# frobelbest/BANet

Measured on AMD Instinct MI355X. Metric: LM iterations/sec (2-frame 640x480 5-level dense BA, 128-coeff depth basis, batch 32), higher is better.
Workload: dtype f32 (SYRK: fp32 operands as bf16x3 / scaled fp16x2 pieces, fp32 accumulate, <= 2e-7 per entry; roofline.syrk_form)

## Files before the change

banet_amd/csrc/api.hip:

```cpp
#include "kernels.hpp"

namespace banet {

static bool aligned256(const void* p) { return (reinterpret_cast<uintptr_t>(p) & 255u) == 0; }

static int check_level(const banet_level_t* lv) {
  if (!lv || !lv->src || !lv->tgt || !lv->depth) return BANET_ERR_INVALID_ARG;
  if (lv->variant < BANET_LEGACY_LM || lv->variant > BANET_BUNDLE) return BANET_ERR_INVALID_ARG;
  if (lv->K > 0 && !lv->basis) return BANET_ERR_INVALID_ARG;
  if ((lv->variant == BANET_BUNDLE) != (lv->K > 0)) return BANET_ERR_INVALID_ARG;
  if (lv->pairs < 0 || (lv->policy != BANET_POLICY_THROUGHPUT && lv->policy != BANET_POLICY_BATCH_INVARIANT)) return BANET_ERR_INVALID_ARG;
  if (lv->pairs > 1 && lv->variant != BANET_BUNDLE && lv->variant != BANET_BUNDLE_CAMERA) return BANET_ERR_INVALID_ARG;
  if (lv->dense) {
    if (!lv->intr || !(lv->scale > 0.f)) return BANET_ERR_INVALID_ARG;
  } else {
    if (!lv->rays || !lv->fx || !lv->fy || !lv->ox || !lv->oy) return BANET_ERR_INVALID_ARG;
  }
  return BANET_OK;
}

static LevelWs carve_level(const banet_level_t* lv, const AsmPlan& pl, void* ws) {
  LevelWs w;
  char* p = static_cast<char*>(ws);
  Arena ar;
// ... 58 lines not shown


constexpr int kRoleSmallLevel = 19200;

int lm_level_plan(const banet_level_t* lv, const banet_mlp_t* mlp, float l2_base, int max_iters, int early_termination,
                  const banet_lm_params_t* params, const banet_state_t* st, void* ws, size_t ws_bytes, LevelRun* run) {
  int rc = check_level(lv);
  if (rc != BANET_OK) return rc;
  rc = check_state(lv, mlp, st);
  if (rc != BANET_OK) return rc;
  if (max_iters < 0) return BANET_ERR_INVALID_ARG;
  AsmPlan& pl = run->pl;
  rc = plan_assemble(lv, num_cus(), &pl);
  if (rc != BANET_OK) return rc;
  if (!ws || !aligned256(ws)) return BANET_ERR_WORKSPACE;
  LevelWs& w = run->w;
  w = carve_level(lv, pl, ws);
  if (ws_bytes < w.total) return BANET_ERR_WORKSPACE;
  SolveArgs& a = run->a;
  a = make_solve_args(lv, mlp, l2_base, w.AtA, w.Atb, w.absres, w.nvalid, st);
  a.max_iters = max_iters;
  a.bigA = w.bigA;
  if (params) {
    if (params->solver != BANET_SOLVER_QR && params->solver != BANET_SOLVER_INVERSE) return BANET_ERR_INVALID_ARG;
    if (!(params->angle_change >= 0.f) || !(params->translation_change >= 0.f) || !(params->residual_ratio > 0.f))
      return BANET_ERR_INVALID_ARG;
    a.lm = *params;
  }
  run->lv = lv;
  run->mlp = mlp;
  run->max_iters = max_iters;
  run->lm = early_termination && lv->variant == BANET_LEGACY_LM;
  run->role = false;
  if (run->lm) {
    a.ctl = w.ctl;
  } else {
    a.queue = assemble_queue(pl, w.partials);
    a.nqueue = 8 * npairs(lv);
    const int Bsel = selection_batch(lv);
    run->role = lv->variant == BANET_BUNDLE && mlp != nullptr && a.use_mlp && syrk_runs_mlp_role(pl.s) && lv->C <= 256 &&
                (lv->C & 3) == 0 && ((long long)Bsel * (pl.s.Gs + 1) <= num_cus() || (Bsel <= 8 && pl.s.Gs >= 16) ||
                 (lv->N <= kRoleSmallLevel && pl.s.Gs >= 4)) &&
                !(lv->flags & kDevMlpInSolve);
    if (run->role) {
      a.mlp_y = w.mlp_y;
      if ((long long)Bsel * (pl.s.Gs + 1) > num_cus()) pl.s.Gs -= 1;
    }
  }
  return BANET_OK;
}

int lm_level_enqueue(const LevelRun& run, hipStream_t s) {
  const banet_level_t* lv = run.lv;
  const AsmPlan& pl = run.pl;
  const LevelWs& w = run.w;
  const SolveArgs& a = run.a;
  const banet_state_t* st = &a.st;
  const int max_iters = run.max_iters;
  int rc;
  if (run.lm) {
    launch_ctl_init(w.ctl, st->iters, lv->B, s);
    const int stride = (int)(sizeof(LmCtl) / sizeof(int32_t));
    for (int it = 0; it <= max_iters; ++it) {
      rc = launch_assemble(lv, pl, st->R, st->T, st->Wc, &w.ctl->active, stride, w.partials, w.AtA, w.Atb, w.absres,
                           w.nvalid, s);
      if (rc != BANET_OK) return rc;
      {
        RangeScope r("solve", lv->N);
        rc = launch_solve(a, s);
      }
      if (rc != BANET_OK) return rc;
    }
  } else {
    launch_zero_iters(st->iters, lv->B, s);
    if (a.queue) launch_zero_iters(a.queue, lv->B * a.nqueue, s);
    const bool role = run.role;
    const banet_mlp_t* mlp = run.mlp;
    for (int it = 0; it < max_iters; ++it) {
      rc = launch_assemble(lv, pl, st->R, st->T, st->Wc, nullptr, 0, w.partials, w.AtA, w.Atb, w.absres, w.nvalid, s,
                           a.queue == nullptr, role ? mlp : nullptr, role ? w.mlp_y : nullptr, nullptr,
                           pl.s.f16 ? (it == 0 ? (max_iters > 1 ? 2 : 0) : 1) : -1);
      if (rc != BANET_OK) return rc;
      {
        RangeScope r("solve", lv->N);
        rc = launch_solve(a, s);
      }
      if (rc != BANET_OK) return rc;
    }
  }
  return BANET_OK;
}

}

using namespace banet;

extern "C" {

int banet_version(void) { return BANET_VERSION; }

const char* banet_error_string(int code) {
  switch (code) {
    case BANET_OK: return "ok";
    case BANET_ERR_INVALID_ARG: return "invalid argument";
    case BANET_ERR_WORKSPACE: return "workspace too small or misaligned";
    case BANET_ERR_UNSUPPORTED: return "shape not supported by the compiled kernel set";
    case BANET_ERR_LAUNCH: return "kernel launch failed";
    default: return "unknown error";
  }
}

size_t banet_equation_construction_workspace_bytes(int B, int N, int C, int P) {
  EqPlan pl;
  if (plan_eq(B, N, C, P, &pl) != BANET_OK) return 0;
// ... 323 lines not shown
```

banet_amd/csrc/assemble.hip:

```cpp
#include <atomic>
#include <dlfcn.h>

#include <cstdio>
#include <cstdlib>
#include <vector>

#include "kernels.hpp"

namespace banet {

namespace {
struct Profiler {
  bool on = false;
  std::vector<hipEvent_t> ev;
  std::vector<int> tag;
  int used = 0;
} g_prof;

struct Timed {
  hipStream_t s;
  int slot;
  Timed(hipStream_t st, int tag) : s(st), slot(-1) {
    if (g_prof.on && (size_t)(2 * g_prof.used + 1) < g_prof.ev.size()) {
      slot = g_prof.used++;
// ... 87 lines not shown

int num_cus() {
  constexpr int kMaxDev = 64, kDefault = 256;
  static std::atomic<int> cached[kMaxDev];
  static const int pinned = [] {
    const char* e = std::getenv("BANET_NUM_CUS");
    const int v = e ? std::atoi(e) : 0;
    return v > 0 && v <= 4096 ? v : 0;
  }();
  if (pinned) return pinned;
  int dev = 0;
  if (hipGetDevice(&dev) != hipSuccess || dev < 0 || dev >= kMaxDev) {
    (void)hipGetLastError();
    return kDefault;
  }
  int n = cached[dev].load(std::memory_order_relaxed);
  if (n == 0) {
    if (hipDeviceGetAttribute(&n, hipDeviceAttributeMultiprocessorCount, dev) != hipSuccess || n <= 0) {
      (void)hipGetLastError();
      n = kDefault;
    }
    cached[dev].store(n, std::memory_order_relaxed);
  }
  return n;
}

int* assemble_queue(const AsmPlan& pl, void* ws) {
  return pl.g.c128 ? reinterpret_cast<int*>(static_cast<char*>(ws) + pl.g.off_queue) : nullptr;
}

int launch_assemble(const banet_level_t* lv, const AsmPlan& pl, const float* R, const float* T, const float* Wc,
                    const int32_t* active, int active_stride, void* ws, float* AtA, float* Atb, float* absres,
                    float* nvalid, hipStream_t s, bool reset_queue, const banet_mlp_t* role_mlp, float* role_y,
                    unsigned char* mask_out, int f16_stats) {
  char* base = static_cast<char*>(ws);
  float* gpart = reinterpret_cast<float*>(base);
  float* rec = lv->K > 0 ? reinterpret_cast<float*>(base + pl.off_rec) : nullptr;
  float* spart = lv->K > 0 ? reinterpret_cast<float*>(base + pl.off_spart) : nullptr;
  int rc;
  if (reset_queue) prepare_gather(lv, pl.g, gpart, s);
  {
    RangeScope r("gather", lv->N);
    Timed t(s, lv->N);
    rc = launch_gather(lv, pl.g, R, T, Wc, active, active_stride, rec, gpart, s, mask_out);
  }
  if (rc != BANET_OK) return rc;
  const float* gred;
  {
    RangeScope r("fold", lv->N);
    gred = finish_gather(lv, pl.g, active, active_stride, gpart, s);
  }
  if (lv->K > 0) {
    RangeScope r("syrk", lv->N);
    Timed t(s, -lv->N);
    MlpRole mr{};
    if (role_mlp != nullptr && role_y != nullptr && syrk_runs_mlp_role(pl.s)) {
      mr.gpart = gred;
      mr.grows = pl.g.frows;
      mr.gstride = pl.g.pstride;
      mr.mlp = *role_mlp;
      mr.C = lv->C;
      mr.pairs = npairs(lv);
      mr.Nf = (float)lv->N * (float)npairs(lv);
      mr.y = role_y;
    }
    rc = launch_syrk(lv->basis, rec, lv->B, lv->N, lv->K, npairs(lv), pl.s, active, active_stride, spart, s,
                     mr.y != nullptr ? &mr : nullptr, f16_stats);
    if (rc != BANET_OK) return rc;
  }
  RangeScope r("reduce", lv->N);
  launch_reduce2(gred, pl.g.frows, pl.g.pstride, spart, pl.s.Gs, pl.s.pstride, active, active_stride, lv->B, lv->K, lv->C,
                 npairs(lv), AtA, Atb, absres, nvalid, s);
  return hipGetLastError() == hipSuccess ? BANET_OK : BANET_ERR_LAUNCH;
}

}
```

banet_amd/csrc/gather.hip:

```cpp
#include <algorithm>
#include "gather_common.hpp"

namespace banet {

template <int VEC, int CH, bool GRAD, int KVEC, int KCH>
__global__ __launch_bounds__(kBlock, BANET_GATHER_WAVES) void ba_gather_kernel(const GatherArgs a) {
  __shared__ float sH[kNumWaves][28][64];
  __shared__ float sAbs[kNumWaves][256];
  const banet_level_t& lv = a.lv;
  const int vb = blockIdx.y, g = blockIdx.x;
  const int b = vb / a.pairs;
  if (a.active != nullptr && a.active[(size_t)b * a.active_stride] == 0) return;
  const int tid = threadIdx.x, lane = tid & 63;
  const int w = wave_id();
  const int N = lv.N, C = lv.C, K = lv.K, H = lv.H, W = lv.W;
  const int Ct = GRAD ? 3 * C : C;
  const bool dense = lv.dense != 0;
  const int dbg = lv.flags;
  const float* __restrict__ tgt_b = lv.tgt + (size_t)vb * H * W * Ct;
  const float* __restrict__ src_b = lv.src + (size_t)b * N * C;
  const float* __restrict__ dep_b = lv.depth + (size_t)b * N;
  const float* __restrict__ bas_b = KCH ? lv.basis + (size_t)b * N * K : nullptr;
  float* __restrict__ rec_b = KCH ? a.rec + (size_t)vb * N * 8 : nullptr;

#pragma unroll
  for (int i = 0; i < 28; ++i) sH[w][i][lane] = 0.f;
#ifdef BANET_TIMING
  float tim0 = 0.f, tim1 = 0.f, tim2 = 0.f, tim3 = 0.f;
#endif
  float absd[CH][VEC];
#pragma unroll
  for (int i = 0; i < CH; ++i)
#pragma unroll
    for (int e = 0; e < VEC; ++e) absd[i][e] = 0.f;
// ... 323 lines not shown
  if (tid == 0) {
    float* dp = a.partials + ((size_t)vb * a.G + g) * (kGHdr + C);
    dp[28] = tim0;
    dp[29] = tim1;
    dp[30] = tim2;
    dp[31] = tim3;
  }
#endif

#pragma unroll
  for (int ch = 0; ch < CH; ++ch)
#pragma unroll
    for (int e = 0; e < VEC; ++e) {
      const int c = (ch * 64 + lane) * VEC + e;
      if (c < C) sAbs[w][c] = absd[ch][e];
    }
  __syncthreads();
  float* __restrict__ part = a.partials + ((size_t)vb * a.G + g) * (kGHdr + C);
  if (tid < 4 * 28) {
    const int ww = tid / 28, i = tid - ww * 28;
    float s = 0.f;
    for (int l = 0; l < 64; ++l) s += sH[ww][i][l];
    sH[ww][i][0] = s;
  }
  __syncthreads();
  if (tid < 28) part[tid] = (sH[0][tid][0] + sH[1][tid][0]) + (sH[2][tid][0] + sH[3][tid][0]);
  for (int c = tid; c < C; c += kBlock) part[kGHdr + c] = (sAbs[0][c] + sAbs[1][c]) + (sAbs[2][c] + sAbs[3][c]);
}


__global__ __launch_bounds__(256) void ba_fold_kernel(const float* __restrict__ in, int rows, int stride,
                                                      float* __restrict__ out, int frows, const int32_t* active,
                                                      int active_stride, int pairs) {
  const int b = blockIdx.y, c = blockIdx.x, e = threadIdx.x;
  if (active != nullptr && active[(size_t)(b / pairs) * active_stride] == 0) return;
  if (e >= stride) return;
  const int r0 = c * kFoldRows, r1 = min(rows, r0 + kFoldRows);
  const float* p = in + ((size_t)b * rows + r0) * stride + e;
  float s0 = 0.f, s1 = 0.f, s2 = 0.f, s3 = 0.f;
  int i = 0;
  const int n = r1 - r0;
  for (; i + 3 < n; i += 4) {
    s0 += p[(size_t)(i + 0) * stride];
    s1 += p[(size_t)(i + 1) * stride];
    s2 += p[(size_t)(i + 2) * stride];
    s3 += p[(size_t)(i + 3) * stride];
  }
  for (; i < n; ++i) s0 += p[(size_t)i * stride];
  out[((size_t)b * frows + c) * stride + e] = (s0 + s1) + (s2 + s3);
}

void prepare_gather(const banet_level_t* lv, const GatherPlan& pl, float* partials, hipStream_t s) {
  if (pl.c128) launch_zero_iters(reinterpret_cast<int32_t*>(reinterpret_cast<char*>(partials) + pl.off_queue), lv->B * npairs(lv) * 8, s);
}

const float* finish_gather(const banet_level_t* lv, const GatherPlan& pl, const int32_t* active, int active_stride,
                           float* partials, hipStream_t s) {
  if (pl.frows == pl.rows) return partials;
  float* out = reinterpret_cast<float*>(reinterpret_cast<char*>(partials) + pl.off_fold);
  hipLaunchKernelGGL(ba_fold_kernel, dim3(pl.frows, lv->B * npairs(lv)), dim3(256), 0, s, partials, pl.rows, pl.pstride, out,
                     pl.frows, active, active_stride, npairs(lv));
  return out;
}

template <int VEC, int CH, bool GRAD>
static int launch_k(const GatherArgs& a, int K, hipStream_t s) {
  dim3 grid(a.G, a.lv.B * a.pairs), block(kBlock);
  const bool keven = (K & 1) == 0;
  if (K == 0)
    hipLaunchKernelGGL((ba_gather_kernel<VEC, CH, GRAD, 1, 0>), grid, block, 0, s, a);
  else if (keven && K <= 128)
    hipLaunchKernelGGL((ba_gather_kernel<VEC, CH, GRAD, 2, 1>), grid, block, 0, s, a);
  else if (keven && K <= 256)
    hipLaunchKernelGGL((ba_gather_kernel<VEC, CH, GRAD, 2, 2>), grid, block, 0, s, a);
  else if (K <= 64)
    hipLaunchKernelGGL((ba_gather_kernel<VEC, CH, GRAD, 1, 1>), grid, block, 0, s, a);
  else if (K <= 128)
    hipLaunchKernelGGL((ba_gather_kernel<VEC, CH, GRAD, 1, 2>), grid, block, 0, s, a);
  else
    return BANET_ERR_UNSUPPORTED;
  return BANET_OK;
}
// ... 47 lines not shown
```

banet_amd/csrc/kernels.hpp:

```cpp
#pragma once
#include "common.hpp"
#include "grid_plan.hpp"

namespace banet {

constexpr int kUStrideS = 8;

int num_cus();

void prepare_gather(const banet_level_t* lv, const GatherPlan& pl, float* partials, hipStream_t s);
int launch_gather(const banet_level_t* lv, const GatherPlan& pl, const float* R, const float* T, const float* Wc,
                  const int32_t* active, int active_stride, float* rec, float* partials, hipStream_t s,
                  unsigned char* mask_out = nullptr);
const float* finish_gather(const banet_level_t* lv, const GatherPlan& pl, const int32_t* active, int active_stride,
                           float* partials, hipStream_t s);

struct MlpRole {
  const float* gpart;
  int grows, gstride;
  banet_mlp_t mlp;
  int C, pairs;
  float Nf;
  float* y;
};
int launch_syrk_wide(const float* basis, const float* rec, int B, int N, int K, int pairs, int Gs, int pstride,
                     const int32_t* active, int active_stride, float* partials, float* aux, hipStream_t s,
                     const float* colmax = nullptr, const float* recmax = nullptr);
int launch_syrk(const float* basis, const float* rec, int B, int N, int K, int pairs, const SyrkPlan& pl,
                const int32_t* active, int active_stride, float* partials, hipStream_t s, const MlpRole* mr = nullptr,
                int f16_stats = -1);
inline bool syrk_runs_mlp_role(const SyrkPlan& pl) { return pl.direct == 2; }
void launch_reduce2(const float* gpart, int Gg, int gstride, const float* spart, int Gs, int sstride,
                    const int32_t* active, int active_stride, int B, int K, int C, int pairs, float* AtA, float* Atb,
                    float* absres, float* nvalid, hipStream_t s);

int launch_assemble(const banet_level_t* lv, const AsmPlan& pl, const float* R, const float* T, const float* Wc,
                    const int32_t* active, int active_stride, void* ws, float* AtA, float* Atb, float* absres,
                    float* nvalid, hipStream_t s, bool reset_queue = true, const banet_mlp_t* role_mlp = nullptr,
                    float* role_y = nullptr, unsigned char* mask_out = nullptr, int f16_stats = -1);
int* assemble_queue(const AsmPlan& pl, void* ws);
int profile_ranges(int enable);
struct RangeScope {
  bool on;
  RangeScope(const char* role, int n = -1);
  ~RangeScope();
};
int profile_begin(int max_launches);
int profile_end(int max_tags, int32_t* tag_points, int32_t* tag_launches, double* tag_ms, int32_t* ntags);

int launch_resample(const float* data, const float* warp, float* out, int B, int N, int C, int H, int W, int mode,
                    hipStream_t s);
int launch_target_map(const float* img, float* out, int B, int H, int W, int C, hipStream_t s);
int launch_depth_output(const float* init, const float* basis, const float* Wc, float* out, int B, int N, int K,
                        hipStream_t s);

bool resample_grad_supported(int B, int N, int C, int H, int W);
size_t resample_grad_workspace_bytes(int B, int N, int C, int H, int W);
int launch_resample_grad(const float* data, const float* warp, const float* gout, float* ddata, float* dwarp, int B, int N, int C, int H,
                         int W, int mode, int overwrite, void* ws, hipStream_t s);
size_t depth_output_grad_workspace_bytes(int B, int N, int K);
int launch_depth_output_grad(const float* basis, const float* Wc, const float* gout, float* dinit, float* dbasis, float* dWc, int B,
                             int N, int K, int overwrite, void* ws, hipStream_t s);

int launch_grid_resample(const float* data, int B, int H, int W, int C, int mode, const banet_grid_level_t* levels, int n_levels,
                         hipStream_t s);
int launch_grid_resample_grad(float* ddata, int B, int H, int W, int C, int mode, const banet_grid_level_t* levels, int n_levels,
                              int overwrite, hipStream_t s);

void launch_reduce(const float* partials, int B, int G, int pstride, int P, float* AtA, float* Atb, hipStream_t s);
struct EqPlan {
  int Gr, tiles, pstride, nb;
  int fast;
// ... 63 lines not shown
size_t sample_stats_grad_det_workspace_bytes(int B, int N, int C, int H, int W);
int launch_sample_stats_grad_det(const float* conv1, const float* conv2, const float* px, const float* py, int B, int N, int C,
                                 int H, int W, const float* dstats, const float* dabs, float* dconv1, float* dconv2, float* dpos,
                                 void* ws, hipStream_t s);
int launch_target_map_adjoint(const float* dmap3, float* dimg, int B, int H, int W, int C, int overwrite, hipStream_t s);

bool small_step_supported(int variant, int B, int N, int C, int K, int pairs);
size_t small_step_workspace_bytes(int variant, int B, int N, int C, int K, int pairs);
int launch_small_step_adjoint(int variant, int B, int N, int C, int K, int pairs, float l2_base, const banet_mlp_t* mlp, const float* AtA,
                              const float* Atb, const float* absres, const float* delta, const float* R, const float* T, const float* gR,
                              const float* gT, const float* gW, float* gAtA, float* gAtb, float* gabs, float* dR, float* dT,
                              const banet_mlp_t* gmlp, void* ws, hipStream_t s);

struct LevelWs {
  float* partials;
  float* AtA;
  float* Atb;
  float* absres;
  float* nvalid;
  LmCtl* ctl;
  float* mlp_y;
  float* bigA;
  size_t total;
};
struct LevelRun {
  const banet_level_t* lv;
  const banet_mlp_t* mlp;
  AsmPlan pl;
  LevelWs w;
  SolveArgs a;
  int max_iters;
  bool lm;
  bool role;
};
int lm_level_plan(const banet_level_t* lv, const banet_mlp_t* mlp, float l2_base, int max_iters, int early_termination,
                  const banet_lm_params_t* params, const banet_state_t* st, void* ws, size_t ws_bytes, LevelRun* run);
int lm_level_enqueue(const LevelRun& run, hipStream_t s);

struct TraceRow {
  banet_state_t from, to;
  int nR, nT, K, P;
};
void launch_lm_trace(const TraceRow& row, int B, hipStream_t s);

}
```

banet_amd/csrc/mlp.hpp:

```cpp
#pragma once
#include "kernels.hpp"

namespace banet {

constexpr float kSeluAlpha = 1.6732632423543772848170429916717f;
constexpr float kSeluScale = 1.0507009873554804934193349852946f;

__device__ __forceinline__ float selu(float x) {
  return kSeluScale * (x > 0.f ? x : kSeluAlpha * (expf(x) - 1.f));
}

template <int NT>
__device__ float block_sum_t(float v, float* sred) {
  v = wave_sum(v);
  __syncthreads();
  if ((threadIdx.x & 63) == 0) sred[threadIdx.x >> 6] = v;
  __syncthreads();
  float r = 0.f;
#pragma unroll
  for (int i = 0; i < NT / 64; ++i) r += sred[i];
  return r;
}

template <int NT>
__device__ void mlp_layer_t(const float* in, float* out, const float* __restrict__ Wt, const float* __restrict__ bias,
                          int nin, int nout, int act, float* sPart, float* sred) {
  const int tid = threadIdx.x;
  const int groups = nout >> 2;
  if ((nout & 3) == 0 && groups <= NT && ((reinterpret_cast<uintptr_t>(Wt) & 15) == 0)) {
    int ksplit = NT / groups;
    if (ksplit > nin) ksplit = nin;
    const int q = tid % groups, sl = tid / groups;
    if (sl < ksplit) {
      const int chunk = (nin + ksplit - 1) / ksplit;
// ... 20 lines not shown
    }
    __syncthreads();
  } else if (nout >= 64) {
    for (int o = tid; o < nout; o += NT) {
      float a0 = 0.f, a1 = 0.f, a2 = 0.f, a3 = 0.f;
      int i = 0;
      for (; i + 3 < nin; i += 4) {
        a0 = fmaf(in[i], Wt[(size_t)i * nout + o], a0);
        a1 = fmaf(in[i + 1], Wt[(size_t)(i + 1) * nout + o], a1);
        a2 = fmaf(in[i + 2], Wt[(size_t)(i + 2) * nout + o], a2);
        a3 = fmaf(in[i + 3], Wt[(size_t)(i + 3) * nout + o], a3);
      }
      for (; i < nin; ++i) a0 = fmaf(in[i], Wt[(size_t)i * nout + o], a0);
      const float v = ((a0 + a1) + (a2 + a3)) + bias[o];
      out[o] = act == 0 ? selu(v) : tanhf(v);
    }
    __syncthreads();
  } else {
    for (int o = 0; o < nout; ++o) {
      float a = 0.f;
      for (int i = tid; i < nin; i += NT) a = fmaf(in[i], Wt[(size_t)i * nout + o], a);
      const float s = block_sum_t<NT>(a, sred);
      if (tid == 0) {
        const float v = s + bias[o];
        out[o] = act == 0 ? selu(v) : tanhf(v);
      }
    }
    __syncthreads();
  }
}


constexpr int kMlpRoleFloats = 256 + 1024 + 1024 + 4096 + 32;
__device__ inline void mlp_role_block(const MlpRole& r, int b, float* sm) {
  const int tid = threadIdx.x, C = r.C;
  float* sAvg = sm;
  float* sH0 = sAvg + 256;
  float* sH1 = sH0 + 1024;
  float* sPart = sH1 + 1024;
  float* sRed = sPart + 4096;
  for (int c = tid; c < C; c += 256) {
    float v = 0.f;
    for (int pp = 0; pp < r.pairs; ++pp) {
      const float* p = r.gpart + ((size_t)b * r.pairs + pp) * r.grows * r.gstride + kGHdr + c;
      float s0 = 0.f, s1 = 0.f, s2 = 0.f, s3 = 0.f;
      int i = 0;
      for (; i + 3 < r.grows; i += 4) {
        s0 += p[(size_t)(i + 0) * r.gstride];
        s1 += p[(size_t)(i + 1) * r.gstride];
        s2 += p[(size_t)(i + 2) * r.gstride];
        s3 += p[(size_t)(i + 3) * r.gstride];
      }
      for (; i < r.grows; ++i) s0 += p[(size_t)i * r.gstride];
      v += (s0 + s1) + (s2 + s3);
    }
    sAvg[c] = v / r.Nf;
  }
  __syncthreads();
  mlp_layer_t<256>(sAvg, sH0, r.mlp.w[0], r.mlp.b[0], C, 2 * C, 0, sPart, sRed);
  mlp_layer_t<256>(sH0, sH1, r.mlp.w[1], r.mlp.b[1], 2 * C, 4 * C, 0, sPart, sRed);
  mlp_layer_t<256>(sH1, sH0, r.mlp.w[2], r.mlp.b[2], 4 * C, 2 * C, 0, sPart, sRed);
  mlp_layer_t<256>(sH0, sH1, r.mlp.w[3], r.mlp.b[3], 2 * C, C, 0, sPart, sRed);
  mlp_layer_t<256>(sH1, sH0, r.mlp.w[4], r.mlp.b[4], C, 1, 1, sPart, sRed);
  if (tid == 0) r.y[b] = sH0[0];
}

}
```

banet_amd/csrc/syrk.hip:

```cpp
#include <algorithm>
#include "kernels.hpp"
#include "mlp.hpp"
#include "syrk_split.hpp"

namespace banet {

struct SyrkArgs {
  const float* basis;
  const float* rec;
  const int32_t* active;
  int active_stride;
  float* partials;
  int N, K, Gs, tiles, pstride;
  int pairs;
  int pass;
  MlpRole mr;
  const float* colmax;
  const float* recmax;
};

template <int NB>
__global__ __launch_bounds__(kBlock, NB > 8 ? 1 : 2) void ba_syrk_kernel(const SyrkArgs a) {
  constexpr int PW = NB > 8 ? 2 : 1;
  constexpr int KPAD = NB * 16;
  constexpr int KP = KPAD + 16;
  constexpr int KV = KPAD >= 64 ? KPAD / 64 : 1;
  constexpr int QPR = KPAD / 4;
  constexpr int QT = (kTilePix * QPR + kBlock - 1) / kBlock;
  constexpr int NSLOT = NB + 1;
  extern __shared__ __attribute__((aligned(16))) float smem[];
  float* sB0 = smem;
  float* sU0 = smem + 2 * kTilePix * KP;
  const int b = blockIdx.y, g = blockIdx.x, tid = threadIdx.x, lane = tid & 63;
  if (a.active != nullptr && a.active[(size_t)b * a.active_stride] == 0) return;
  const int w = wave_id();
// ... 773 lines not shown
}

__global__ __launch_bounds__(256) void ba_colmax_kernel(const float* __restrict__ basis, int N, int K, const int32_t* active,
                                                        int active_stride, unsigned* __restrict__ colmax) {
  __shared__ unsigned sMax[256][4];
  const int b = blockIdx.y, tid = threadIdx.x;
  if (active != nullptr && active[(size_t)b * active_stride] == 0) return;
  const int QK = K >> 2;
  const int cq = tid % QK, r0 = tid / QK, rstep = 256 / QK;
  const float* bas_b = basis + (size_t)b * N * K;
  f32x4 mx = {0.f, 0.f, 0.f, 0.f};
  const int rows_per_block = (N + gridDim.x - 1) / gridDim.x;
  const int n0 = blockIdx.x * rows_per_block, n1 = min(N, n0 + rows_per_block);
  for (int n = n0 + r0; n < n1; n += rstep) {
    const f32x4 v = __builtin_nontemporal_load(reinterpret_cast<const f32x4*>(bas_b + (size_t)n * K + 4 * cq));
#pragma unroll
    for (int e = 0; e < 4; ++e) mx[e] = (fabsf(v[e]) > mx[e] || v[e] != v[e]) ? fabsf(v[e]) : mx[e];
  }
#pragma unroll
  for (int e = 0; e < 4; ++e) sMax[tid][e] = __float_as_uint(mx[e]);
  __syncthreads();
  if (tid < QK) {
    unsigned m[4] = {0u, 0u, 0u, 0u};
    for (int r = 0; r < rstep; ++r)
#pragma unroll
      for (int e = 0; e < 4; ++e) m[e] = max(m[e], sMax[r * QK + tid][e]);
#pragma unroll
    for (int e = 0; e < 4; ++e) atomicMax(&colmax[(size_t)b * K + 4 * tid + e], m[e]);
  }
}

__global__ __launch_bounds__(256) void ba_recmax_kernel(const float* __restrict__ rec, int N, int pairs, const int32_t* active,
                                                        int active_stride, float* __restrict__ out) {
  __shared__ float sRed[4][2];
  const int b = blockIdx.y, tid = threadIdx.x;
  if (active != nullptr && active[(size_t)b * active_stride] == 0) return;
  const float* rec_b = rec + (size_t)b * pairs * N * 8;
  float smx = 0.f, wmx = 0.f;
  for (int n = blockIdx.x * 256 + tid; n < N; n += gridDim.x * 256) {
    float ssum = 0.f, w2 = 0.f;
    for (int p = 0; p < pairs; ++p) {
      const float4 ua = *reinterpret_cast<const float4*>(rec_b + ((size_t)p * N + n) * 8);
      const float4 ub = *reinterpret_cast<const float4*>(rec_b + ((size_t)p * N + n) * 8 + 4);
      ssum += ub.z;
      w2 = fmaxf(w2, fmaxf(fmaxf(ua.x * ua.x, ua.y * ua.y), fmaxf(ua.z * ua.z, ua.w * ua.w)));
      w2 = fmaxf(w2, fmaxf(fmaxf(ub.x * ub.x, ub.y * ub.y), ub.w * ub.w));
      if (ua.x != ua.x || ua.y != ua.y || ua.z != ua.z || ua.w != ua.w || ub.x != ub.x || ub.y != ub.y || ub.z != ub.z || ub.w != ub.w)
        w2 = __builtin_nanf("");
    }
    const float q = ssum > 0.f ? w2 / ssum : (w2 != w2 ? w2 : 0.f);
    smx = (ssum > smx || ssum != ssum) ? ssum : smx;
    wmx = (q > wmx || q != q) ? q : wmx;
  }
  auto nanmax = [](float a_, float b_) { return (a_ != a_) ? a_ : (b_ != b_) ? b_ : fmaxf(a_, b_); };
#pragma unroll
  for (int sh = 1; sh < 64; sh <<= 1) {
    smx = nanmax(smx, __shfl_xor(smx, sh, 64));
    wmx = nanmax(wmx, __shfl_xor(wmx, sh, 64));
  }
  if ((tid & 63) == 0) {
    sRed[tid >> 6][0] = smx;
    sRed[tid >> 6][1] = wmx;
  }
  __syncthreads();
  if (tid == 0) {
    out[((size_t)b * kRecMaxBlocks + blockIdx.x) * 2] = nanmax(nanmax(sRed[0][0], sRed[1][0]), nanmax(sRed[2][0], sRed[3][0]));
    out[((size_t)b * kRecMaxBlocks + blockIdx.x) * 2 + 1] = nanmax(nanmax(sRed[0][1], sRed[1][1]), nanmax(sRed[2][1], sRed[3][1]));
  }
}


template <int NB>
static void launch_syrk_nb(const SyrkArgs& a, int B, hipStream_t s) {
  constexpr int KPAD = NB * 16, KP = KPAD + 16;
  size_t fl = (size_t)2 * kTilePix * KP + 2 * kTilePix * kUStrideS;
  const size_t epi = (size_t)4 * 8 * KPAD;
  if (fl < epi) fl = epi;
  const size_t lds = fl * sizeof(float);
  auto k = ba_syrk_kernel<NB>;
  if (lds > 64 * 1024) (void)hipFuncSetAttribute((const void*)k, hipFuncAttributeMaxDynamicSharedMemorySize, (int)lds);
  hipLaunchKernelGGL(k, dim3(a.Gs, B), dim3(kBlock), lds, s, a);
}

template <int KH, int T0>
static void launch_bf16x6(const SyrkArgs& a, int B, hipStream_t s) {
  const dim3 grid(a.Gs + (a.mr.y != nullptr ? 1 : 0), B), block(kBlock);
  switch (a.pairs) {
    case 1: hipLaunchKernelGGL((ba_syrk_bf16x6_kernel<KH, 1, T0>), grid, block, 0, s, a); break;
    case 2: hipLaunchKernelGGL((ba_syrk_bf16x6_kernel<KH, 2, T0>), grid, block, 0, s, a); break;
    case 3: hipLaunchKernelGGL((ba_syrk_bf16x6_kernel<KH, 3, T0>), grid, block, 0, s, a); break;
    default: hipLaunchKernelGGL((ba_syrk_bf16x6_kernel<KH, 4, T0>), grid, block, 0, s, a); break;
  }
}

template <int KH>
static void launch_direct(const SyrkArgs& a, int B, hipStream_t s) {
  const dim3 grid(a.Gs, B), block(kBlock);
  switch (a.pairs) {
    case 1: hipLaunchKernelGGL((ba_syrk_direct_kernel<KH, 1>), grid, block, 0, s, a); break;
    case 2: hipLaunchKernelGGL((ba_syrk_direct_kernel<KH, 2>), grid, block, 0, s, a); break;
    case 3: hipLaunchKernelGGL((ba_syrk_direct_kernel<KH, 3>), grid, block, 0, s, a); break;
    default: hipLaunchKernelGGL((ba_syrk_direct_kernel<KH, 4>), grid, block, 0, s, a); break;
  }
}

int launch_syrk(const float* basis, const float* rec, int B, int N, int K, int pairs, const SyrkPlan& pl,
                const int32_t* active, int active_stride, float* partials, hipStream_t s, const MlpRole* mr, int f16_stats) {
  if (pl.direct == 3) {
    const float* colmax_w = nullptr;
    float* recmax_w = nullptr;
    if (pl.f16 && f16_stats >= 0) {
      unsigned* cm = reinterpret_cast<unsigned*>(reinterpret_cast<char*>(partials) + pl.off_colmax);
      recmax_w = reinterpret_cast<float*>(reinterpret_cast<char*>(partials) + pl.off_recmax);
      if (f16_stats != 1) {
        launch_zero_iters(reinterpret_cast<int32_t*>(cm), B * K, s);
        const int G = std::max(1, std::min((N + 255) / 256, (8 * num_cus() + B - 1) / B));
        hipLaunchKernelGGL(ba_colmax_kernel, dim3(G, B), dim3(256), 0, s, basis, N, K, active, active_stride, cm);
      }
      hipLaunchKernelGGL(ba_recmax_kernel, dim3(kRecMaxBlocks, B), dim3(256), 0, s, rec, N, pairs, active, active_stride, recmax_w);
      colmax_w = reinterpret_cast<const float*>(cm);
    }
    return launch_syrk_wide(basis, rec, B, N, K, pairs, pl.Gs, pl.pstride, active, active_stride, partials,
                            reinterpret_cast<float*>(reinterpret_cast<char*>(partials) + pl.off_aux), s, colmax_w, recmax_w);
  }
  SyrkArgs a{basis, rec, active, active_stride, partials, N, K, pl.Gs, pl.tiles, pl.pstride, pairs, 0, MlpRole{}, nullptr, nullptr};
  if (pl.direct == 2) {
    if (mr != nullptr) a.mr = *mr;
    if (pl.f16 && f16_stats == 2) {
      unsigned* colmax = reinterpret_cast<unsigned*>(reinterpret_cast<char*>(partials) + pl.off_colmax);
      launch_zero_iters(reinterpret_cast<int32_t*>(colmax), B * K, s);
      a.colmax = reinterpret_cast<const float*>(colmax);
      if (K == 128)
        launch_bf16x6<2, 1>(a, B, s);
      else
        launch_bf16x6<1, 1>(a, B, s);
      return hipGetLastError() == hipSuccess ? BANET_OK : BANET_ERR_LAUNCH;
    }
    if (pl.f16 && f16_stats >= 0) {
      unsigned* colmax = reinterpret_cast<unsigned*>(reinterpret_cast<char*>(partials) + pl.off_colmax);
      float* recmax = reinterpret_cast<float*>(reinterpret_cast<char*>(partials) + pl.off_recmax);
      if (f16_stats == 0) {
        launch_zero_iters(reinterpret_cast<int32_t*>(colmax), B * K, s);
        const int G = std::max(1, std::min((N + 255) / 256, (8 * num_cus() + B - 1) / B));
        hipLaunchKernelGGL(ba_colmax_kernel, dim3(G, B), dim3(256), 0, s, basis, N, K, active, active_stride, colmax);
      }
      hipLaunchKernelGGL(ba_recmax_kernel, dim3(kRecMaxBlocks, B), dim3(256), 0, s, rec, N, pairs, active, active_stride, recmax);
      a.colmax = reinterpret_cast<const float*>(colmax);
      a.recmax = recmax;
      if (K == 128)
        launch_bf16x6<2, 16>(a, B, s);
      else
        launch_bf16x6<1, 16>(a, B, s);
      return hipGetLastError() == hipSuccess ? BANET_OK : BANET_ERR_LAUNCH;
    }
    if (K == 128) {
      if (pl.x3)
        launch_bf16x6<2, 3>(a, B, s);
      else
        launch_bf16x6<2, 0>(a, B, s);
    } else {
      launch_bf16x6<1, 0>(a, B, s);
    }
    return hipGetLastError() == hipSuccess ? BANET_OK : BANET_ERR_LAUNCH;
  }
  if (pl.direct) {
    if (K == 128)
      launch_direct<2>(a, B, s);
    else
      launch_direct<1>(a, B, s);
    return hipGetLastError() == hipSuccess ? BANET_OK : BANET_ERR_LAUNCH;
  }
  for (int pass = 0; pass < pairs; ++pass) {
    a.pass = pass;
    switch (pl.nb) {
      case 1: launch_syrk_nb<1>(a, B, s); break;
      case 2: launch_syrk_nb<2>(a, B, s); break;
      case 4: launch_syrk_nb<4>(a, B, s); break;
      case 8: launch_syrk_nb<8>(a, B, s); break;
      case 16: launch_syrk_nb<16>(a, B, s); break;
// ... 16 lines not shown
```

Before: 24710.

## Merge fold, recmax and MLP role into one pre-SYRK kernel launch

Adds a combined pre_syrk kernel whose grid holds MLP-role blocks, recmax blocks and fold blocks, replacing separate fold and recmax launches before the SYRK. When the MLP role cannot run inside SYRK, it now runs in this pre-kernel, reading raw unfolded partials and folding them through LDS staging. The goal is fewer kernel launches and idle gaps per LM iteration. In exchange the role blocks do extra reads of unfolded rows, and the heterogeneous block mix may be load-imbalanced.

```diff
diff --git a/banet_amd/csrc/api.hip b/banet_amd/csrc/api.hip
--- a/banet_amd/csrc/api.hip
+++ b/banet_amd/csrc/api.hip
@@ -114,20 +114,25 @@
   run->max_iters = max_iters;
   run->lm = early_termination && lv->variant == BANET_LEGACY_LM;
   run->role = false;
+  run->role_pre = false;
   if (run->lm) {
     a.ctl = w.ctl;
   } else {
     a.queue = assemble_queue(pl, w.partials);
     a.nqueue = 8 * npairs(lv);
     const int Bsel = selection_batch(lv);
-    run->role = lv->variant == BANET_BUNDLE && mlp != nullptr && a.use_mlp && syrk_runs_mlp_role(pl.s) && lv->C <= 256 &&
-                (lv->C & 3) == 0 && ((long long)Bsel * (pl.s.Gs + 1) <= num_cus() || (Bsel <= 8 && pl.s.Gs >= 16) ||
-                 (lv->N <= kRoleSmallLevel && pl.s.Gs >= 4)) &&
-                !(lv->flags & kDevMlpInSolve);
+    const bool can_role = lv->variant == BANET_BUNDLE && mlp != nullptr && a.use_mlp && syrk_runs_mlp_role(pl.s) && lv->C <= 256 &&
+                          (lv->C & 3) == 0 && !(lv->flags & kDevMlpInSolve);
+    run->role = can_role && ((long long)Bsel * (pl.s.Gs + 1) <= num_cus() || (Bsel <= 8 && pl.s.Gs >= 16) ||
+                             (lv->N <= kRoleSmallLevel && pl.s.Gs >= 4));
     if (run->role) {
       a.mlp_y = w.mlp_y;
       if ((long long)Bsel * (pl.s.Gs + 1) > num_cus()) pl.s.Gs -= 1;
     }
+#ifndef BANET_PRE_SYRK_SPLIT
+    run->role_pre = can_role && !run->role;
+    if (run->role_pre) a.mlp_y = w.mlp_y;
+#endif
   }
   return BANET_OK;
 }
@@ -156,12 +161,12 @@
   } else {
     launch_zero_iters(st->iters, lv->B, s);
     if (a.queue) launch_zero_iters(a.queue, lv->B * a.nqueue, s);
-    const bool role = run.role;
+    const bool role = run.role || run.role_pre;
     const banet_mlp_t* mlp = run.mlp;
     for (int it = 0; it < max_iters; ++it) {
       rc = launch_assemble(lv, pl, st->R, st->T, st->Wc, nullptr, 0, w.partials, w.AtA, w.Atb, w.absres, w.nvalid, s,
                            a.queue == nullptr, role ? mlp : nullptr, role ? w.mlp_y : nullptr, nullptr,
-                           pl.s.f16 ? (it == 0 ? (max_iters > 1 ? 2 : 0) : 1) : -1);
+                           pl.s.f16 ? (it == 0 ? (max_iters > 1 ? 2 : 0) : 1) : -1, run.role_pre);
       if (rc != BANET_OK) return rc;
       {
         RangeScope r("solve", lv->N);
diff --git a/banet_amd/csrc/assemble.hip b/banet_amd/csrc/assemble.hip
--- a/banet_amd/csrc/assemble.hip
+++ b/banet_amd/csrc/assemble.hip
@@ -143,7 +143,7 @@
 int launch_assemble(const banet_level_t* lv, const AsmPlan& pl, const float* R, const float* T, const float* Wc,
                     const int32_t* active, int active_stride, void* ws, float* AtA, float* Atb, float* absres,
                     float* nvalid, hipStream_t s, bool reset_queue, const banet_mlp_t* role_mlp, float* role_y,
-                    unsigned char* mask_out, int f16_stats) {
+                    unsigned char* mask_out, int f16_stats, bool role_pre) {
   char* base = static_cast<char*>(ws);
   float* gpart = reinterpret_cast<float*>(base);
   float* rec = lv->K > 0 ? reinterpret_cast<float*>(base + pl.off_rec) : nullptr;
@@ -156,27 +156,43 @@
     rc = launch_gather(lv, pl.g, R, T, Wc, active, active_stride, rec, gpart, s, mask_out);
   }
   if (rc != BANET_OK) return rc;
+  const int pairs = npairs(lv);
+  const bool fold = pl.g.frows != pl.g.rows;
+  const bool recmax = lv->K > 0 && syrk_reads_recmax(pl.s, f16_stats);
+  MlpRole mr{};
+  if (lv->K > 0 && role_mlp != nullptr && role_y != nullptr && syrk_runs_mlp_role(pl.s)) {
+    mr.gpart = fold && !role_pre ? reinterpret_cast<const float*>(base + pl.g.off_fold) : gpart;
+    mr.grows = fold && role_pre ? pl.g.rows : pl.g.frows;
+    mr.gstride = pl.g.pstride;
+    mr.mlp = *role_mlp;
+    mr.C = lv->C;
+    mr.pairs = pairs;
+    mr.Nf = (float)lv->N * (float)pairs;
+    mr.y = role_y;
+  }
+  const bool pre_role = mr.y != nullptr && role_pre;
+#ifdef BANET_PRE_SYRK_SPLIT
+  const bool merged = pre_role;
+#else
+  const bool merged = pre_role || (fold && recmax);
+#endif
   const float* gred;
-  {
+  if (merged) {
+    RangeScope r("pre_syrk", lv->N);
+    gred = fold ? reinterpret_cast<const float*>(base + pl.g.off_fold) : gpart;
+    rc = launch_pre_syrk(pl.g, lv->B, lv->N, pairs, gpart, rec,
+                         recmax ? reinterpret_cast<float*>(reinterpret_cast<char*>(spart) + pl.s.off_recmax) : nullptr,
+                         pre_role ? &mr : nullptr, active, active_stride, s);
+    if (rc != BANET_OK) return rc;
+  } else {
     RangeScope r("fold", lv->N);
     gred = finish_gather(lv, pl.g, active, active_stride, gpart, s);
   }
   if (lv->K > 0) {
     RangeScope r("syrk", lv->N);
     Timed t(s, -lv->N);
-    MlpRole mr{};
-    if (role_mlp != nullptr && role_y != nullptr && syrk_runs_mlp_role(pl.s)) {
-      mr.gpart = gred;
-      mr.grows = pl.g.frows;
-      mr.gstride = pl.g.pstride;
-      mr.mlp = *role_mlp;
-      mr.C = lv->C;
-      mr.pairs = npairs(lv);
-      mr.Nf = (float)lv->N * (float)npairs(lv);
-      mr.y = role_y;
-    }
-    rc = launch_syrk(lv->basis, rec, lv->B, lv->N, lv->K, npairs(lv), pl.s, active, active_stride, spart, s,
-                     mr.y != nullptr ? &mr : nullptr, f16_stats);
+    rc = launch_syrk(lv->basis, rec, lv->B, lv->N, lv->K, pairs, pl.s, active, active_stride, spart, s,
+                     mr.y != nullptr && !pre_role ? &mr : nullptr, f16_stats, merged && recmax);
     if (rc != BANET_OK) return rc;
   }
   RangeScope r("reduce", lv->N);
diff --git a/banet_amd/csrc/gather.hip b/banet_amd/csrc/gather.hip
--- a/banet_amd/csrc/gather.hip
+++ b/banet_amd/csrc/gather.hip
@@ -1,5 +1,6 @@
 #include <algorithm>
 #include "gather_common.hpp"
+#include "pre_syrk.hpp"
 
 namespace banet {
 
@@ -389,22 +390,7 @@
 __global__ __launch_bounds__(256) void ba_fold_kernel(const float* __restrict__ in, int rows, int stride,
                                                       float* __restrict__ out, int frows, const int32_t* active,
                                                       int active_stride, int pairs) {
-  const int b = blockIdx.y, c = blockIdx.x, e = threadIdx.x;
-  if (active != nullptr && active[(size_t)(b / pairs) * active_stride] == 0) return;
-  if (e >= stride) return;
-  const int r0 = c * kFoldRows, r1 = min(rows, r0 + kFoldRows);
-  const float* p = in + ((size_t)b * rows + r0) * stride + e;
-  float s0 = 0.f, s1 = 0.f, s2 = 0.f, s3 = 0.f;
-  int i = 0;
-  const int n = r1 - r0;
-  for (; i + 3 < n; i += 4) {
-    s0 += p[(size_t)(i + 0) * stride];
-    s1 += p[(size_t)(i + 1) * stride];
-    s2 += p[(size_t)(i + 2) * stride];
-    s3 += p[(size_t)(i + 3) * stride];
-  }
-  for (; i < n; ++i) s0 += p[(size_t)i * stride];
-  out[((size_t)b * frows + c) * stride + e] = (s0 + s1) + (s2 + s3);
+  fold_block(in, rows, stride, out, frows, active, active_stride, pairs, blockIdx.y, blockIdx.x);
 }
 
 void prepare_gather(const banet_level_t* lv, const GatherPlan& pl, float* partials, hipStream_t s) {
diff --git a/banet_amd/csrc/kernels.hpp b/banet_amd/csrc/kernels.hpp
--- a/banet_amd/csrc/kernels.hpp
+++ b/banet_amd/csrc/kernels.hpp
@@ -28,16 +28,24 @@
                      const float* colmax = nullptr, const float* recmax = nullptr);
 int launch_syrk(const float* basis, const float* rec, int B, int N, int K, int pairs, const SyrkPlan& pl,
                 const int32_t* active, int active_stride, float* partials, hipStream_t s, const MlpRole* mr = nullptr,
-                int f16_stats = -1);
+                int f16_stats = -1,
+                bool recmax_in_place = false);
+inline bool syrk_reads_recmax(const SyrkPlan& pl, int f16_stats) {
+  return pl.f16 && f16_stats >= 0 && (pl.direct == 3 || (pl.direct == 2 && f16_stats != 2));
+}
 inline bool syrk_runs_mlp_role(const SyrkPlan& pl) { return pl.direct == 2; }
 void launch_reduce2(const float* gpart, int Gg, int gstride, const float* spart, int Gs, int sstride,
                     const int32_t* active, int active_stride, int B, int K, int C, int pairs, float* AtA, float* Atb,
                     float* absres, float* nvalid, hipStream_t s);
 
+int launch_pre_syrk(const GatherPlan& g, int B, int N, int pairs, const float* gpart, const float* rec, float* recmax,
+                    const MlpRole* mr, const int32_t* active, int active_stride, hipStream_t s);
+
 int launch_assemble(const banet_level_t* lv, const AsmPlan& pl, const float* R, const float* T, const float* Wc,
                     const int32_t* active, int active_stride, void* ws, float* AtA, float* Atb, float* absres,
                     float* nvalid, hipStream_t s, bool reset_queue = true, const banet_mlp_t* role_mlp = nullptr,
-                    float* role_y = nullptr, unsigned char* mask_out = nullptr, int f16_stats = -1);
+                    float* role_y = nullptr, unsigned char* mask_out = nullptr, int f16_stats = -1,
+                    bool role_pre = false);
 int* assemble_queue(const AsmPlan& pl, void* ws);
 int profile_ranges(int enable);
 struct RangeScope {
@@ -167,6 +175,7 @@
   int max_iters;
   bool lm;
   bool role;
+  bool role_pre;
 };
 int lm_level_plan(const banet_level_t* lv, const banet_mlp_t* mlp, float l2_base, int max_iters, int early_termination,
                   const banet_lm_params_t* params, const banet_state_t* st, void* ws, size_t ws_bytes, LevelRun* run);
diff --git a/banet_amd/csrc/mlp.hpp b/banet_amd/csrc/mlp.hpp
--- a/banet_amd/csrc/mlp.hpp
+++ b/banet_amd/csrc/mlp.hpp
@@ -1,5 +1,6 @@
 #pragma once
 #include "kernels.hpp"
+#include "pre_syrk.hpp"
 
 namespace banet {
 
@@ -86,13 +87,8 @@
 
 
 constexpr int kMlpRoleFloats = 256 + 1024 + 1024 + 4096 + 32;
-__device__ inline void mlp_role_block(const MlpRole& r, int b, float* sm) {
+__device__ inline void mlp_role_avg(const MlpRole& r, int b, float* sAvg) {
   const int tid = threadIdx.x, C = r.C;
-  float* sAvg = sm;
-  float* sH0 = sAvg + 256;
-  float* sH1 = sH0 + 1024;
-  float* sPart = sH1 + 1024;
-  float* sRed = sPart + 4096;
   for (int c = tid; c < C; c += 256) {
     float v = 0.f;
     for (int pp = 0; pp < r.pairs; ++pp) {
@@ -111,6 +107,53 @@
     sAvg[c] = v / r.Nf;
   }
   __syncthreads();
+}
+
+__device__ inline void mlp_role_avg_raw(const MlpRole& r, int b, float* sAvg, float* sStage) {
+  const int tid = threadIdx.x, C = r.C, QC = C >> 2;
+  const int frows = (r.grows + kFoldRows - 1) / kFoldRows, f4 = frows & ~3;
+  const int q = tid % QC, slot = tid / QC, slots = 256 / QC;
+  const int chunk = (4096 / C) & ~3;
+  float v = 0.f;
+  for (int pp = 0; pp < r.pairs; ++pp) {
+    const float* p = r.gpart + ((size_t)b * r.pairs + pp) * r.grows * r.gstride + kGHdr;
+    float s0 = 0.f, s1 = 0.f, s2 = 0.f, s3 = 0.f;
+    for (int g0 = 0; g0 < frows; g0 += chunk) {
+      const int gn = min(chunk, frows - g0);
+      if (slot < slots)
+        for (int j = slot; j < gn; j += slots) {
+          const int r0 = (g0 + j) * kFoldRows;
+          *reinterpret_cast<float4*>(sStage + j * C + 4 * q) =
+              fold_rows_sum<float4>(p + (size_t)r0 * r.gstride + 4 * q, min(kFoldRows, r.grows - r0), r.gstride);
+        }
+      __syncthreads();
+      if (tid < C) {
+        int j = 0;
+        for (; j + 3 < gn && g0 + j + 3 < f4; j += 4) {
+          s0 += sStage[(j + 0) * C + tid];
+          s1 += sStage[(j + 1) * C + tid];
+          s2 += sStage[(j + 2) * C + tid];
+          s3 += sStage[(j + 3) * C + tid];
+        }
+        for (; j < gn; ++j) s0 += sStage[j * C + tid];
+      }
+      __syncthreads();
+    }
+    v += (s0 + s1) + (s2 + s3);
+  }
+  if (tid < C) sAvg[tid] = v / r.Nf;
+  __syncthreads();
+}
+
+__device__ inline void mlp_role_block(const MlpRole& r, int b, float* sm, bool raw = false) {
+  const int tid = threadIdx.x, C = r.C;
+  float* sAvg = sm;
+  float* sH0 = sAvg + 256;
+  float* sH1 = sH0 + 1024;
+  float* sPart = sH1 + 1024;
+  float* sRed = sPart + 4096;
+  if (raw) mlp_role_avg_raw(r, b, sAvg, sPart);
+  else mlp_role_avg(r, b, sAvg);
   mlp_layer_t<256>(sAvg, sH0, r.mlp.w[0], r.mlp.b[0], C, 2 * C, 0, sPart, sRed);
   mlp_layer_t<256>(sH0, sH1, r.mlp.w[1], r.mlp.b[1], 2 * C, 4 * C, 0, sPart, sRed);
   mlp_layer_t<256>(sH1, sH0, r.mlp.w[2], r.mlp.b[2], 4 * C, 2 * C, 0, sPart, sRed);
diff --git a/banet_amd/csrc/pre_syrk.hip b/banet_amd/csrc/pre_syrk.hip
--- /dev/null
+++ b/banet_amd/csrc/pre_syrk.hip
@@ -0,0 +1,62 @@
+#include "kernels.hpp"
+#include "mlp.hpp"
+#include "pre_syrk.hpp"
+
+namespace banet {
+
+struct PreSyrkArgs {
+  const float* gpart;
+  float* fold_out;
+  const float* rec;
+  float* recmax;
+  const int32_t* active;
+  int active_stride;
+  int rows, frows, gstride, pairs, N;
+  int nrole, nrec;
+  int role_raw;
+  MlpRole mr;
+};
+
+__global__ __launch_bounds__(256) void ba_pre_syrk_kernel(const PreSyrkArgs a) {
+  extern __shared__ __align__(16) float sPre[];
+  int i = blockIdx.x;
+  if (i < a.nrole) {
+    if (a.active != nullptr && a.active[(size_t)i * a.active_stride] == 0) return;
+    mlp_role_block(a.mr, i, sPre, a.role_raw != 0);
+    return;
+  }
+  i -= a.nrole;
+  if (i < a.nrec) {
+    recmax_block(a.rec, a.N, a.pairs, a.active, a.active_stride, a.recmax, i / kRecMaxBlocks, i % kRecMaxBlocks, kRecMaxBlocks, sPre);
+    return;
+  }
+  i -= a.nrec;
+  fold_block(a.gpart, a.rows, a.gstride, a.fold_out, a.frows, a.active, a.active_stride, a.pairs, i / a.frows, i % a.frows);
+}
+
+int launch_pre_syrk(const GatherPlan& g, int B, int N, int pairs, const float* gpart, const float* rec, float* recmax,
+                    const MlpRole* mr, const int32_t* active, int active_stride, hipStream_t s) {
+  const bool fold = g.frows != g.rows;
+  PreSyrkArgs a{};
+  a.gpart = gpart;
+  a.fold_out = fold ? reinterpret_cast<float*>(reinterpret_cast<char*>(const_cast<float*>(gpart)) + g.off_fold) : nullptr;
+  a.rec = rec;
+  a.recmax = recmax;
+  a.active = active;
+  a.active_stride = active_stride;
+  a.rows = g.rows;
+  a.frows = g.frows;
+  a.gstride = g.pstride;
+  a.pairs = pairs;
+  a.N = N;
+  a.nrole = mr != nullptr ? B : 0;
+  a.nrec = recmax != nullptr ? kRecMaxBlocks * B : 0;
+  a.role_raw = fold ? 1 : 0;
+  if (mr != nullptr) a.mr = *mr;
+  const int nfold = fold ? g.frows * B * pairs : 0;
+  const size_t lds = (a.nrole ? kMlpRoleFloats : 8) * sizeof(float);
+  hipLaunchKernelGGL(ba_pre_syrk_kernel, dim3(a.nrole + a.nrec + nfold), dim3(256), lds, s, a);
+  return hipGetLastError() == hipSuccess ? BANET_OK : BANET_ERR_LAUNCH;
+}
+
+}
diff --git a/banet_amd/csrc/pre_syrk.hpp b/banet_amd/csrc/pre_syrk.hpp
--- /dev/null
+++ b/banet_amd/csrc/pre_syrk.hpp
@@ -0,0 +1,79 @@
+#pragma once
+#include "common.hpp"
+
+namespace banet {
+
+template <class T>
+__device__ __forceinline__ T fold_rows_sum(const float* p, int n, int stride) {
+  T s0{}, s1{}, s2{}, s3{};
+  int i = 0;
+  for (; i + 15 < n; i += 16) {
+    T v[16];
+#pragma unroll
+    for (int k = 0; k < 16; ++k) v[k] = *reinterpret_cast<const T*>(p + (size_t)(i + k) * stride);
+#pragma unroll
+    for (int k = 0; k < 16; k += 4) {
+      s0 += v[k + 0];
+      s1 += v[k + 1];
+      s2 += v[k + 2];
+      s3 += v[k + 3];
+    }
+  }
+  for (; i + 3 < n; i += 4) {
+    s0 += *reinterpret_cast<const T*>(p + (size_t)(i + 0) * stride);
+    s1 += *reinterpret_cast<const T*>(p + (size_t)(i + 1) * stride);
+    s2 += *reinterpret_cast<const T*>(p + (size_t)(i + 2) * stride);
+    s3 += *reinterpret_cast<const T*>(p + (size_t)(i + 3) * stride);
+  }
+  for (; i < n; ++i) s0 += *reinterpret_cast<const T*>(p + (size_t)i * stride);
+  return (s0 + s1) + (s2 + s3);
+}
+
+__device__ __forceinline__ void fold_block(const float* __restrict__ in, int rows, int stride, float* __restrict__ out, int frows,
+                                           const int32_t* active, int active_stride, int pairs, int b, int c) {
+  const int e = threadIdx.x;
+  if (active != nullptr && active[(size_t)(b / pairs) * active_stride] == 0) return;
+  if (e >= stride) return;
+  const int r0 = c * kFoldRows, r1 = min(rows, r0 + kFoldRows);
+  out[((size_t)b * frows + c) * stride + e] = fold_rows_sum<float>(in + ((size_t)b * rows + r0) * stride + e, r1 - r0, stride);
+}
+
+__device__ __forceinline__ void recmax_block(const float* __restrict__ rec, int N, int pairs, const int32_t* active,
+                                             int active_stride, float* __restrict__ out, int b, int bx, int nbx, float* sRed) {
+  const int tid = threadIdx.x;
+  if (active != nullptr && active[(size_t)b * active_stride] == 0) return;
+  const float* rec_b = rec + (size_t)b * pairs * N * 8;
+  float smx = 0.f, wmx = 0.f;
+  for (int n = bx * 256 + tid; n < N; n += nbx * 256) {
+    float ssum = 0.f, w2 = 0.f;
+    for (int p = 0; p < pairs; ++p) {
+      const float4 ua = *reinterpret_cast<const float4*>(rec_b + ((size_t)p * N + n) * 8);
+      const float4 ub = *reinterpret_cast<const float4*>(rec_b + ((size_t)p * N + n) * 8 + 4);
+      ssum += ub.z;
+      w2 = fmaxf(w2, fmaxf(fmaxf(ua.x * ua.x, ua.y * ua.y), fmaxf(ua.z * ua.z, ua.w * ua.w)));
+      w2 = fmaxf(w2, fmaxf(fmaxf(ub.x * ub.x, ub.y * ub.y), ub.w * ub.w));
+      if (ua.x != ua.x || ua.y != ua.y || ua.z != ua.z || ua.w != ua.w || ub.x != ub.x || ub.y != ub.y || ub.z != ub.z || ub.w != ub.w)
+        w2 = __builtin_nanf("");
+    }
+    const float q = ssum > 0.f ? w2 / ssum : (w2 != w2 ? w2 : 0.f);
+    smx = (ssum > smx || ssum != ssum) ? ssum : smx;
+    wmx = (q > wmx || q != q) ? q : wmx;
+  }
+  auto nanmax = [](float a_, float b_) { return (a_ != a_) ? a_ : (b_ != b_) ? b_ : fmaxf(a_, b_); };
+#pragma unroll
+  for (int sh = 1; sh < 64; sh <<= 1) {
+    smx = nanmax(smx, __shfl_xor(smx, sh, 64));
+    wmx = nanmax(wmx, __shfl_xor(wmx, sh, 64));
+  }
+  if ((tid & 63) == 0) {
+    sRed[2 * (tid >> 6)] = smx;
+    sRed[2 * (tid >> 6) + 1] = wmx;
+  }
+  __syncthreads();
+  if (tid == 0) {
+    out[((size_t)b * kRecMaxBlocks + bx) * 2] = nanmax(nanmax(sRed[0], sRed[2]), nanmax(sRed[4], sRed[6]));
+    out[((size_t)b * kRecMaxBlocks + bx) * 2 + 1] = nanmax(nanmax(sRed[1], sRed[3]), nanmax(sRed[5], sRed[7]));
+  }
+}
+
+}
diff --git a/banet_amd/csrc/syrk.hip b/banet_amd/csrc/syrk.hip
--- a/banet_amd/csrc/syrk.hip
+++ b/banet_amd/csrc/syrk.hip
@@ -1,6 +1,7 @@
 #include <algorithm>
 #include "kernels.hpp"
 #include "mlp.hpp"
+#include "pre_syrk.hpp"
 #include "syrk_split.hpp"
 
 namespace banet {
@@ -840,41 +841,8 @@
 
 __global__ __launch_bounds__(256) void ba_recmax_kernel(const float* __restrict__ rec, int N, int pairs, const int32_t* active,
                                                         int active_stride, float* __restrict__ out) {
-  __shared__ float sRed[4][2];
-  const int b = blockIdx.y, tid = threadIdx.x;
-  if (active != nullptr && active[(size_t)b * active_stride] == 0) return;
-  const float* rec_b = rec + (size_t)b * pairs * N * 8;
-  float smx = 0.f, wmx = 0.f;
-  for (int n = blockIdx.x * 256 + tid; n < N; n += gridDim.x * 256) {
-    float ssum = 0.f, w2 = 0.f;
-    for (int p = 0; p < pairs; ++p) {
-      const float4 ua = *reinterpret_cast<const float4*>(rec_b + ((size_t)p * N + n) * 8);
-      const float4 ub = *reinterpret_cast<const float4*>(rec_b + ((size_t)p * N + n) * 8 + 4);
-      ssum += ub.z;
-      w2 = fmaxf(w2, fmaxf(fmaxf(ua.x * ua.x, ua.y * ua.y), fmaxf(ua.z * ua.z, ua.w * ua.w)));
-      w2 = fmaxf(w2, fmaxf(fmaxf(ub.x * ub.x, ub.y * ub.y), ub.w * ub.w));
-      if (ua.x != ua.x || ua.y != ua.y || ua.z != ua.z || ua.w != ua.w || ub.x != ub.x || ub.y != ub.y || ub.z != ub.z || ub.w != ub.w)
-        w2 = __builtin_nanf("");
-    }
-    const float q = ssum > 0.f ? w2 / ssum : (w2 != w2 ? w2 : 0.f);
-    smx = (ssum > smx || ssum != ssum) ? ssum : smx;
-    wmx = (q > wmx || q != q) ? q : wmx;
-  }
-  auto nanmax = [](float a_, float b_) { return (a_ != a_) ? a_ : (b_ != b_) ? b_ : fmaxf(a_, b_); };
-#pragma unroll
-  for (int sh = 1; sh < 64; sh <<= 1) {
-    smx = nanmax(smx, __shfl_xor(smx, sh, 64));
-    wmx = nanmax(wmx, __shfl_xor(wmx, sh, 64));
-  }
-  if ((tid & 63) == 0) {
-    sRed[tid >> 6][0] = smx;
-    sRed[tid >> 6][1] = wmx;
-  }
-  __syncthreads();
-  if (tid == 0) {
-    out[((size_t)b * kRecMaxBlocks + blockIdx.x) * 2] = nanmax(nanmax(sRed[0][0], sRed[1][0]), nanmax(sRed[2][0], sRed[3][0]));
-    out[((size_t)b * kRecMaxBlocks + blockIdx.x) * 2 + 1] = nanmax(nanmax(sRed[0][1], sRed[1][1]), nanmax(sRed[2][1], sRed[3][1]));
-  }
+  __shared__ float sRed[8];
+  recmax_block(rec, N, pairs, active, active_stride, out, blockIdx.y, blockIdx.x, gridDim.x, sRed);
 }
 
 
@@ -913,7 +881,8 @@
 }
 
 int launch_syrk(const float* basis, const float* rec, int B, int N, int K, int pairs, const SyrkPlan& pl,
-                const int32_t* active, int active_stride, float* partials, hipStream_t s, const MlpRole* mr, int f16_stats) {
+                const int32_t* active, int active_stride, float* partials, hipStream_t s, const MlpRole* mr, int f16_stats,
+                bool recmax_in_place) {
   if (pl.direct == 3) {
     const float* colmax_w = nullptr;
     float* recmax_w = nullptr;
@@ -925,7 +894,8 @@
         const int G = std::max(1, std::min((N + 255) / 256, (8 * num_cus() + B - 1) / B));
         hipLaunchKernelGGL(ba_colmax_kernel, dim3(G, B), dim3(256), 0, s, basis, N, K, active, active_stride, cm);
       }
-      hipLaunchKernelGGL(ba_recmax_kernel, dim3(kRecMaxBlocks, B), dim3(256), 0, s, rec, N, pairs, active, active_stride, recmax_w);
+      if (!recmax_in_place)
+        hipLaunchKernelGGL(ba_recmax_kernel, dim3(kRecMaxBlocks, B), dim3(256), 0, s, rec, N, pairs, active, active_stride, recmax_w);
       colmax_w = reinterpret_cast<const float*>(cm);
     }
     return launch_syrk_wide(basis, rec, B, N, K, pairs, pl.Gs, pl.pstride, active, active_stride, partials,
@@ -952,7 +922,8 @@
         const int G = std::max(1, std::min((N + 255) / 256, (8 * num_cus() + B - 1) / B));
         hipLaunchKernelGGL(ba_colmax_kernel, dim3(G, B), dim3(256), 0, s, basis, N, K, active, active_stride, colmax);
       }
-      hipLaunchKernelGGL(ba_recmax_kernel, dim3(kRecMaxBlocks, B), dim3(256), 0, s, rec, N, pairs, active, active_stride, recmax);
+      if (!recmax_in_place)
+        hipLaunchKernelGGL(ba_recmax_kernel, dim3(kRecMaxBlocks, B), dim3(256), 0, s, rec, N, pairs, active, active_stride, recmax);
       a.colmax = reinterpret_cast<const float*>(colmax);
       a.recmax = recmax;
       if (K == 128)
```

Result: no change. 24820 (median of 6 runs) (+0.5%).
